# stoneMo/DeepAVFusion

Measured on AMD Instinct MI355X. Metric: AV-pairs/sec, DeepAVFusion ViT-B pre-training step (224px + 10s audio, image mask 0.75), higher is better.
Workload: dtype bf16; 1 GPU; AVMAE(DeepAVFusion base) fwd+bwd+allreduce+AdamW, B=64/GPU, 224x224 RGB + (128,640) log-mel, masks 0.75/0.8, fusion attn_ratio 0.25 mlp_ratio 1.0; global_batch=64, parallelism=dp1, graph=True

## Files before the change

### deepavfusion_amd/_lib.py

```python
from __future__ import annotations

import ctypes as C
import os

import torch

_HERE = os.path.dirname(os.path.abspath(__file__))
LIB_PATH = os.path.join(_HERE, 'libdavfusion_hip.so')

_p, _i, _l, _f, _sz = C.c_void_p, C.c_int, C.c_long, C.c_float, C.c_size_t

ABI_VERSION = 9

SIGNATURES = {
    'dav_abi_version': [],
    'dav_build_flags': [],
    'dav_last_error_string': [],
    'dav_tune': [_i, _i],
    'dav_gemm_nt_bf16': [_p, _p, _i, _i, _i, _i, _i, _p, _p, _i, _p, _i, _p, _i, _p, _p, _p, _i, _i, _p, _p, _i, _i, _i, _f, _i, _p],
    'dav_gemm_nt_ln_bf16': [_p, _p, _i, _i, _i, _i, _i, _p, _p, _i, _p, _i, _p, _i, _p, _p, _p, _i, _i, _p, _p, _i, _i, _i, _f, _i, _p, _p],
    'dav_ln_fold_grouped': [_p, _i, _p],
    'dav_rowstats_cast': [_p, _l, _i, _i, _i, _p, _p, _p],
    'dav_layernorm_bwd_twin': [_p, _l, _p, _i, _p, _l, _p, _i, _i, _i, _f, _p, _p, _p, _p,
                               _p, _l, _i, _p, _l, _p, _l,
                               _p, _l, _i, _p, _l, _p, _l,
                               _p, _p, _p, _p, _sz, _p],
    'dav_nt_issue_log': [_i, _p, _i],
    'dav_nt_tune_set': [_p, _i],
    'dav_gemm_tn_bf16': [_p, _p, _i, _i, _i, _i, _i, _p, _p, _p, _i, _i, _p, _i, _p],
    'dav_gemm_tn_grouped_bf16': [_p, _i, _p],
    'dav_gemm_tn_gang_workspace_bytes': [_p, _i],
    'dav_gemm_tn_gang_bf16': [_p, _i, _p, _sz, _p],
    'dav_gemm_tn_grouped_bf16_gated': [_p, _i, _p, _p],
    'dav_gemm_tn_gang_bf16_gated': [_p, _i, _p, _sz, _p, _p],
    'dav_attn_fwd': [_p, _p, _p, _p, _p, _i, _i, _i, _i, _i, _i, _l, _i, _l, _i, _l, _i, _l, _i, _f, _p],
    'dav_attn_bwd': [_p] * 10 + [_i] * 6 + [_l, _i] * 8 + [_f, _p],
    'dav_attn_bwd_part': [_p] * 10 + [_i] * 6 + [_l, _i] * 8 + [_f, _i, _p],
    'dav_add_cast': [_p, _p, _p, _p, _l, _p],
    'dav_attn_bwd_ctx': [_p] * 10 + [_i] * 6 + [_l, _i] * 8 + [_f, _i, _i, _p],
    'dav_attn_bias_fwd': [_p, _p, _p, _p, _p, _i, _i, _i, _i, _i, _i, _l, _i, _l, _i, _l, _i, _l, _i, _f, _p, _i, _i, _p],
    'dav_attn_bias_bwd': [_p] * 10 + [_i] * 6 + [_l, _i] * 8 + [_f, _p, _i, _i, _p, _i, _p],
    'dav_attn_drop_fwd': [_p, _p, _p, _p, _p, _i, _i, _i, _i, _i, _i, _l, _i, _l, _i, _l, _i, _l, _i, _f, _p, _i, _f, _p],
    'dav_attn_drop_bwd': [_p] * 10 + [_i] * 6 + [_l, _i] * 8 + [_f, _p, _i, _f, _i, _i, _p],
    'dav_window_unfold': [_p, _i, _p, _i, _i, _i, _i, _i, _i, _f, _p, _i, _p],
    'dav_window_fold': [_p, _p, _p, _i, _i, _i, _i, _i, _i, _f, _p, _p],
    'dav_relpos_bias_build': [_p, _p, _p, _i, _i, _i, _i, _i, _f, _p, _p],
    'dav_relpos_bias_bwd': [_p, _p, _i, _i, _i, _i, _i, _i, _p, _p],
    'dav_layernorm_fwd': [_p, _l, _i, _p, _l, _i, _i, _i, _p, _p, _f, _p, _p, _p, _p, _p],
    'dav_layernorm_bwd': [_p, _l, _i, _p, _l, _i, _i, _i, _p, _p, _p, _p, _p,
                          _p, _l, _i, _p, _l, _p, _l,
                          _p, _l, _i, _p, _l, _p, _l,
                          _p, _p, _p, _sz, _p],
    'dav_layernorm_bwd_workspace_bytes': [_i, _i],
    'dav_layernorm_bwd_reduce_grouped': [_p, _i, _p],
    'dav_mask_build': [_p, _i, _i, _i, _p, _p, _p, _p, _p, _p],
    'dav_patch_gather': [_p, _i, _i, _i, _i, _p, _i, _p, _p],
    'dav_patch_gather3d': [_p, _i, _i, _i, _i, _i, _i, _p, _i, _p, _p],
    'dav_unshuffle_fwd': [_p, _p, _p, _p, _i, _i, _i, _i, _p, _l, _i, _p],
    'dav_rows_gather_cast': [_p, _l, _i, _p, _i, _i, _i, _p, _p],
    'dav_rows_axpy': [_p, _p, _p, _i, _i, _i, _p, _p],
    'dav_rows_scale_cast': [_p, _p, _i, _i, _i, _p, _p],
    'dav_dropout_rows': [_p, _i, _p, _p, _f, _p, _i, _i, _i, _p, _i, _p],
    'dav_unshuffle_bwd_reduce': [_p, _l, _i, _p, _i, _i, _i, _i, _p, _p, _p],
    'dav_patch_mse_fwd': [_p, _p, _p, _i, _i, _i, _i, _i, _p, _p, _p, _p, _p, _p],
    'dav_patch_mse_bwd': [_p, _p, _p, _p, _p, _p, _p, _i, _i, _i, _i, _p, _p],
    'dav_pair_expand': [_p, _p, _i, _i, _i, _i, _p, _p],
    'dav_pair_reduce': [_p, _i, _i, _i, _i, _p, _p, _p],
# ... 27 lines not shown
    'dav_batch_suspend': [_i],
    'dav_batch_end': [],
    'dav_batch_abort': [],
    'dav_batch_stats': [_p, _p],
    'dav_adamw_flat': [_p, _p, _p, _p, _p, _l, _p, _p, _i, _f, _f, _f, _p, _f, _p, _i, _p, _p, _p],
    'dav_step_guard': [_p, _p, _p, _f, _f, _p, _p, _p],
    'dav_cast_transpose_grouped': [_p, _i, _p],
}

class DavLnReduce(C.Structure):
    _fields_ = [('workspace', C.c_void_p), ('dgamma', C.c_void_p), ('dbeta', C.c_void_p), ('rows', C.c_int), ('D', C.c_int)]


class DavNtLn(C.Structure):
    _fields_ = [('stats', C.c_void_p), ('stats2', C.c_void_p), ('A2', C.c_void_p), ('ln_c', C.c_void_p), ('eps', C.c_float),
                ('a_r0', C.c_int), ('a_r1', C.c_int), ('stats_out', C.c_void_p), ('twin_out', C.c_void_p), ('ld_twin', C.c_int)]


class DavLnFold(C.Structure):
    _fields_ = [('w', C.c_void_p), ('gamma', C.c_void_p), ('beta', C.c_void_p), ('bias', C.c_void_p),
                ('w_ln_bf16', C.c_void_p), ('ln_c', C.c_void_p), ('ln_d', C.c_void_p), ('N', C.c_int), ('K', C.c_int)]


class DavTranspose(C.Structure):
    _fields_ = [('x', C.c_void_p), ('y_bf16', C.c_void_p), ('R', C.c_int), ('C', C.c_int)]


class DavTnProblem(C.Structure):
    _fields_ = [('A', C.c_void_p), ('B', C.c_void_p), ('C', C.c_void_p), ('bias_grad', C.c_void_p),
                ('Mc', C.c_int), ('N', C.c_int), ('K', C.c_int), ('lda', C.c_int), ('ldb', C.c_int), ('ldc', C.c_int),
                ('a_rowmap', C.c_int * 3), ('b_rowmap', C.c_int * 3), ('flags', C.c_int)]


ERRORS = {-1: 'bad shape', -2: 'unsupported dtype', -3: 'insufficient workspace', -4: 'HIP error', -5: 'misaligned pointer/stride'}

_lib = None


def load():
    global _lib
    if _lib is not None:
        return _lib
    if not os.path.exists(LIB_PATH):
        raise RuntimeError(f'{LIB_PATH} is missing: the DeepAVFusion HIP kernels are not built '
                           '(run __graft_entry__.build() or make -C deepavfusion_amd/csrc). There is no CPU fallback.')
    lib = C.CDLL(LIB_PATH)
    for name, argtypes in SIGNATURES.items():
        fn = getattr(lib, name)
        fn.argtypes = argtypes
        fn.restype = _sz if name.endswith('workspace_bytes') else (C.c_char_p if name == 'dav_last_error_string' else _i)
    if lib.dav_abi_version() != ABI_VERSION:
        raise RuntimeError('libdavfusion_hip.so ABI version mismatch')
    _lib = lib
    load_nt_tuning(NT_TUNING_PATH)
    return lib


def kernel_source_hash():
    import glob
    import hashlib
    here = os.path.dirname(os.path.abspath(__file__))
    h = hashlib.sha1()
    for f in sorted(glob.glob(os.path.join(here, 'csrc', '*.hip')) + glob.glob(os.path.join(here, 'csrc', '*.h'))) + [os.path.join(here, 'tuning', 'nt_gfx950.json')]:
        h.update(os.path.basename(f).encode())
        h.update(open(f, 'rb').read())
    return h.hexdigest()[:16]
# ... 29 lines not shown
```

### deepavfusion_amd/csrc/accum/gemm_tn_gated.hip

```cpp
#include "../gemm.hip"

namespace {

static_assert(sizeof(TGWrite) + sizeof(const int*) <= 4096, "kernel argument block");
constexpr int TG_BETA_WORD = (int)(offsetof(TNParams, beta) / 4), TG_PROB_WORDS = (int)(sizeof(TNParams) / 4);

__global__ __launch_bounds__(64) void gemm_tn_gang_write_gated_kernel(const TGWrite w, const int* __restrict__ write_gate) {
  TGHeader* hd = reinterpret_cast<TGHeader*>(w.ws);
  TNParams* probs = reinterpret_cast<TNParams*>(w.ws + sizeof(TGHeader));
  TGDesc* desc = reinterpret_cast<TGDesc*>(w.ws + sizeof(TGHeader) + (size_t)w.count_total * sizeof(TNParams));
  const int b = blockIdx.x, t = threadIdx.x;
  if (b < w.item_count) {
    const TGItem it = w.item[b];
    const int nr = it.nrnc >> 16, nc = it.nrnc & 0xffff, r0 = it.r0c0 >> 16, c0 = it.r0c0 & 0xffff;
    for (int i = t; i < nr * nc; i += 64) desc[it.desc_first + i] = TGDesc{it.prob, ((r0 + i / nc) << 16) | (c0 + i % nc)};
    return;
  }
  const bool closed = write_gate[0] == 0;
  const int* src = reinterpret_cast<const int*>(w.prob);
  int* dst = reinterpret_cast<int*>(probs + w.prob_first);
  for (int i = t; i < w.prob_count * TG_PROB_WORDS; i += 64) dst[i] = (closed && i % TG_PROB_WORDS == TG_BETA_WORD) ? 1 : src[i];
  if (w.write_header) {
    if (t < 8) hd->head[t] = 0;
    if (t < 9) hd->q_start[t] = w.q_start[t];
// ... 86 lines not shown
  for (int i = 0; i < count; ++i) {
    if (w.prob_count == TG_WCH) { flush(); reset(i); }
    const DavTnProblem& q = probs[i];
    TNParams& p = w.prob[w.prob_count++];
    p.A = (const bf16_t*)q.A; p.B = (const bf16_t*)q.B; p.Mc = q.Mc; p.N = q.N; p.K = q.K; p.lda = q.lda; p.ldb = q.ldb;
    p.amap = RowMap{q.a_rowmap[0], q.a_rowmap[1], q.a_rowmap[2]};
    p.bmap = RowMap{q.b_rowmap[0], q.b_rowmap[1], q.b_rowmap[2]};
    p.C = q.C; p.ldc = q.ldc; p.beta = (q.flags & 1) ? 0 : 1; p.bias_grad = q.bias_grad; p.debug_plain_store = 0; p.splits = 1;
    for (const TGPlanItem* it : by_prob[i]) {
      if (w.item_count == TG_WIT) { flush(); reset(i + 1); }
      w.item[w.item_count++] = TGItem{i, q_start[it->queue] + it->first, (it->r0 << 16) | it->c0, (it->nr << 16) | it->nc};
    }
  }
  flush();
  static std::mutex dev_mu;
  static int dev_cus[64] = {0};
  int n_wg = 256;
  {
    int dev = 0;
    if (hipGetDevice(&dev) != hipSuccess || dev < 0 || dev >= 64) return DAV_ERR_HIP;
    std::lock_guard<std::mutex> lk(dev_mu);
    if (!dev_cus[dev]) {
      if (hipFuncSetAttribute((const void*)gemm_tn_gang_kernel, hipFuncAttributeMaxDynamicSharedMemorySize, 160 * 1024) != hipSuccess) return DAV_ERR_HIP;
      int cus = 256;
      (void)hipDeviceGetAttribute(&cus, hipDeviceAttributeMultiprocessorCount, dev);
      dev_cus[dev] = cus > 0 ? cus : 256;
    }
    n_wg = dev_cus[dev];
  }
  const int grid = (int)std::min<long>(n_wg, (long)q_start[8]);
  DAV_LAUNCH(gemm_tn_gang_kernel, dim3(grid), dim3(512), TNG_LDS, stream, (char*)workspace, count, dbg);
  return dav_launch_status();
}
```

### deepavfusion_amd/engine.py

```python
from __future__ import annotations

import os
from typing import Callable, Dict, List, Optional

import torch

from . import ops
from .ops import F32

BF16 = torch.bfloat16
PRECISION = 'bf16'


def set_precision(p: str):
    global BF16, PRECISION
    if p not in ('bf16', 'fp32'):
        raise ValueError(p)
    PRECISION = p
    BF16 = torch.float32 if p == 'fp32' else torch.bfloat16

_GRAD_READY: Optional[Callable[[torch.nn.Parameter], None]] = None


def set_grad_ready_hook(fn: Optional[Callable[[torch.nn.Parameter], None]]):
# ... 324 lines not shown
            _FOLD_PENDING.clear()
            _FOLD_JOINED.clear()
        _FOLD_SCOPE = self.prev
        return False


class region:

    def __enter__(self):
        self.own = None
        if _BATCH is not None:
            ops.batch_region(True)
        elif batching_allowed():
            self.own = batch(auto_lanes=True)
            self.own.__enter__()
        return self

    def __exit__(self, et, ev, tb):
        if self.own is not None:
            return self.own.__exit__(et, ev, tb)
        if _BATCH is not None and et is None:
            ops.batch_region(False)
        return False


WGRAD_GANG = os.environ.get('DAV_WGRAD_GANG', '1') != '0'
WGRAD_GANG_MIN_TILES = 512
WGRAD_MERGE = int(os.environ.get('DAV_WGRAD_MERGE', '0'))
WGRAD_FLUSH_LAYERS = None


WGRAD_EAGER_DP_MERGE = 3


def wgrad_flush_due(layer: int, depth: int) -> bool:
    if not WGRAD_GANG or layer == 0 or layer in (WGRAD_FLUSH_LAYERS or ()):
        return True
    if WGRAD_MERGE > 0:
        return (depth - layer) % WGRAD_MERGE == 0
    return _GRAD_READY is not None and WGRAD_FLUSH_LAYERS is None and (depth - layer) % WGRAD_EAGER_DP_MERGE == 0


_DEFERRED = None
_DEFERRED_LN = None
_DEFERRED_LN_READY = []


class deferred_wgrads:
    def __enter__(self):
        global _DEFERRED, _DEFERRED_LN
        self.prev = (_DEFERRED, _DEFERRED_LN)
        _DEFERRED, _DEFERRED_LN = [], []
        return self

    def __exit__(self, *exc):
        global _DEFERRED, _DEFERRED_LN
        if exc[0] is None:
            flush_wgrads()
        _DEFERRED, _DEFERRED_LN = self.prev


_OVERWRITE = None


def wgrad_overwrite_begin(gate=None):
    global _OVERWRITE
    _OVERWRITE = dict(written=set(), touched=set(), params={}, gate=gate)


def wgrad_overwrite_end():
    global _OVERWRITE
    st, _OVERWRITE = _OVERWRITE, None
    return list(st['params'].values()) if st else []


def deferred_operands_to(stream):
    for pr in (_DEFERRED or []):
        for k in ('A', 'B'):
            t = pr.get(k)
            if torch.is_tensor(t) and t.is_cuda:
                t.record_stream(stream)
    for item in (_DEFERRED_LN or []):
        if torch.is_tensor(item[0]) and item[0].is_cuda:
            item[0].record_stream(stream)


def flush_wgrads():
    if _DEFERRED_LN:
        items = list(_DEFERRED_LN)
        del _DEFERRED_LN[:]
        ops.layernorm_bwd_reduce_grouped(items)
        for pair in _DEFERRED_LN_READY:
            _ready(*pair)
        del _DEFERRED_LN_READY[:]
    if not _DEFERRED:
        return
    probs = list(_DEFERRED)
    del _DEFERRED[:]
    while probs:
        seen, now, later = set(), [], []
        for pr in probs:
            key = pr['C'].data_ptr()
            (later if key in seen else now).append(pr)
            seen.add(key)
        now.sort(key=lambda pr: -pr['Mc'])
        gate = _OVERWRITE['gate'] if _OVERWRITE is not None else None
        gated = {} if gate is None else {'gate': gate}
        gang = WGRAD_GANG and PRECISION == 'bf16' and (sum(-(-pr['N'] // 256) * -(-pr['K'] // 256) for pr in now) >= WGRAD_GANG_MIN_TILES
                                                       or any(pr['Mc'] % 64 for pr in now))
        if _OVERWRITE is not None:
            for pr in now:
                key = pr['C'].data_ptr()
                pr['overwrite'] = bool(pr.get('weight') is not None and key not in _OVERWRITE['written'] and key not in _OVERWRITE['touched'])
                if gate is not None and (pr['A'].dtype == F32 or (not gang and pr['Mc'] % 64)):
                    pr['overwrite'] = False
                _OVERWRITE['written'].add(key)
                if pr.get('weight') is None:
                    _OVERWRITE['touched'].add(pr.get('gbase', key))
                if pr['overwrite']:
                    _OVERWRITE['params'][id(pr['weight'])] = pr['weight']
        if gang:
            ops.gemm_tn_gang(now, **gated)
        else:
            grouped = [pr for pr in now if pr['Mc'] % 64 == 0 or pr['A'].dtype == F32]
            if grouped:
                ops.gemm_tn_grouped(grouped, **gated)
            for pr in now:
                if pr['Mc'] % 64 and pr['A'].dtype != F32:
                    ops.gemm_tn(pr['A'], pr['B'], pr['Mc'], pr['N'], pr['K'], pr['C'], lda=pr['lda'], ldb=pr['ldb'], ldc=pr['ldc'],
                                a_rowmap=pr.get('a_rowmap'), b_rowmap=pr.get('b_rowmap'), beta=0 if pr.get('overwrite') else 1,
                                bias_grad=pr.get('bias_grad'))
        for pr in now:
            _ready(*pr['ready'])
        probs = later


def ln_fwd(norm, x0, x1, B, eps=None, want_f32=False, want_bf16=True):
    D = norm.weight.shape[0]
    r0 = x0.shape[1] if x0 is not None else 0
    r1 = x1.shape[1] if x1 is not None else 0
    if x0 is None:
        x0, r0, x1, r1 = x1, r1, None, 0
    dev = x0.device
    M = B * (r0 + r1)
    y = _e((M, D), BF16, dev) if want_bf16 else None
    y32 = _e((M, D), F32, dev) if want_f32 else None
    if PRECISION == 'fp32' and y is not None and y32 is not None:
        y32 = y
    mean, rstd = _e((M,), F32, dev), _e((M,), F32, dev)
    ops.layernorm_fwd(x0, r0 * D, r0, x1, r1 * D, r1, B, D, norm.weight, norm.bias, norm.eps if eps is None else eps,
                      y, y32, mean, rstd)
    return y, y32, (mean, rstd)


# ... 854 lines not shown
    else:
        got = (img.shape[2] // pt) * (img.shape[3] // 16) * (img.shape[4] // 16)
        if tuple(img.shape[2:]) != tuple(pe.input_size):
            raise RuntimeError(f'The size of tensor a ({got}) must match the size of tensor b ({L}) at non-singleton dimension 1')
    if C != pe.proj.weight.shape[1]:
        raise RuntimeError(f'Given groups=1, weight of size {list(pe.proj.weight.shape)}, expected input{list(img.shape)} to have '
                           f'{pe.proj.weight.shape[1]} channels, but got {C} channels instead')
    if clip and nk != L:
        raise RuntimeError(f'The size of tensor a ({nk}) must match the size of tensor b ({L}) at non-singleton dimension 1')
    K = C * pt * 256
    A = _e((B * nk, K), BF16, img.device)
    ops.patch_gather(img, ids_keep32, nk, A, pt)
    Wb = wcache(pe.proj.weight)
    tok = _e((B, nk, D), F32, img.device)
    pos_by_id = ids_keep32 is not None and not clip
    if ln_fuse_ok(D) and K % 64 == 0:
        tw = (_e((B * nk, D), BF16, img.device), _e((B * nk, D // 64, 2), F32, img.device))
        ops.gemm_nt_ln(A, Wb, B * nk, D, K, prod=dict(stats_out=tw[1], twin_out=tw[0], ld_twin=D), bias=pe.proj.bias, res=vit.pos_embed,
                       ldres=D, res_rows=ids_keep32 if pos_by_id else None, res_rowmap=None if pos_by_id else (L, 0, 0), C_out=tok)
        tw_set(tok, *tw)
    else:
        ops.gemm_nt(A, Wb, B * nk, D, K, bias=pe.proj.bias, res=vit.pos_embed, ldres=D,
                    res_rows=ids_keep32 if pos_by_id else None, res_rowmap=None if pos_by_id else (L, 0, 0), C_out=tok)
    return tok, dict(A=A, nk=nk)


def patch_embed_bwd(vit, t, g, gb):
    pe = vit.patch_embed
    D = vit.embed_dim
    A = t['A']
    M, K = A.shape
    if gb is None:
        gb = to_bf16(g)
    ops.gemm_tn(gb, A, M, D, K, gbuf(pe.proj.weight).view(D, K), beta=1, bias_grad=gbuf(pe.proj.bias))
    _ready(pe.proj.weight, pe.proj.bias)


def drain(steps):
    try:
        while True:
            next(steps)
    except StopIteration as e:
        return e.value


def decoder_fwd(dec, x_b, xf_b, ids_restore32, B, nk, nF):
    return drain(decoder_fwd_steps(dec, x_b, xf_b, ids_restore32, B, nk, nF))


def decoder_fwd_steps(dec, x_b, xf_b, ids_restore32, B, nk, nF):
    L = ids_restore32.shape[1]
    Dd = dec.embed.weight.shape[0]
    dev = x_b.device
    emb = lin_fwd(dec.embed, x_b, B * nk)
    x = _e((B, nF + L, Dd), F32, dev)
    lin_fwd(dec.embed, xf_b, B * nF, out=x, c_rowmap=(nF, nF + L, 0))
    ops.unshuffle_fwd(emb, dec.mask_token, dec.pos_embed, ids_restore32, B, L, nk, Dd, x, (nF + L) * Dd, nF)
    tapes = []
    swin = getattr(dec, 'arch', 'plain') == 'swin'
    for blk in dec.blocks:
        if swin:
            x, bt = swin_block_fwd(blk, x, nF)
        else:
            x, bt = block_fwd(blk, x, None, dec.heads, blk.norm1.eps)
        tapes.append(bt)
        yield
# ... 152 lines not shown
```

### deepavfusion_amd/ops.py

```python
from __future__ import annotations

import ctypes as C
from typing import Optional, Sequence

import torch

from . import _lib

BF16 = torch.bfloat16
F32 = torch.float32


def _stream():
    return torch.cuda.current_stream().cuda_stream


import threading

_TLS = threading.local()


def hold(*tensors):
    h = getattr(_TLS, 'hold', None)
    if h is not None:
# ... 197 lines not shown
            continue
        _lib.check(lib.dav_gemm_tn_grouped_bf16(_tn_problem_array(chunk), len(chunk), _stream()), 'dav_gemm_tn_grouped_bf16')


def _tn_problem_array(problems):
    arr = (_lib.DavTnProblem * len(problems))()
    for q, d in zip(arr, problems):
        q.A, q.B, q.C, q.bias_grad = _ptr(d['A']), _ptr(d['B']), _ptr(d['C']), _ptr(d.get('bias_grad'))
        q.Mc, q.N, q.K, q.lda, q.ldb, q.ldc = d['Mc'], d['N'], d['K'], d['lda'], d['ldb'], d['ldc']
        q.a_rowmap[:] = d.get('a_rowmap') or (0, 0, 0)
        q.b_rowmap[:] = d.get('b_rowmap') or (0, 0, 0)
        q.flags = 1 if d.get('overwrite') else 0
    return arr


def gemm_tn_gang(problems, workspace_fill=None, gate=None):
    if not problems:
        return
    if problems[0]['A'].dtype == F32:
        return gemm_tn_grouped(problems) if gate is None else gemm_tn_grouped(problems, gate)
    lib = _lib.load()
    arr = _tn_problem_array(problems)
    nbytes = int(lib.dav_gemm_tn_gang_workspace_bytes(arr, len(problems)))
    if nbytes == 0:
        raise RuntimeError('dav_gemm_tn_gang_workspace_bytes: invalid weight-gradient problem (shape / alignment)')
    ws = torch.empty(nbytes, dtype=torch.uint8, device=problems[0]['A'].device)
    if workspace_fill is not None:
        ws.fill_(workspace_fill)
    hold(ws)
    if gate is not None:
        _lib.check(lib.dav_gemm_tn_gang_bf16_gated(arr, len(problems), _ptr(ws), nbytes, _gate_ptr(gate), _stream()), 'dav_gemm_tn_gang_bf16_gated')
        return
    _lib.check(lib.dav_gemm_tn_gang_bf16(arr, len(problems), _ptr(ws), nbytes, _stream()), 'dav_gemm_tn_gang_bf16')


def attn_fwd(q_ptr, k_ptr, v_ptr, O, LSE, B, H, Nq, Nk, dqk, dv, q_bs, q_rs, k_bs, k_rs, v_bs, v_rs, o_bs, o_rs, scale):
    lib = _lib.load()
    if O.dtype == F32:
        _lib.check(lib.dav_attn_fwd_f32(q_ptr, k_ptr, v_ptr, _ptr(O), _ptr(LSE), B, H, Nq, Nk, dqk, dv, q_bs, q_rs, k_bs, k_rs,
                                        v_bs, v_rs, o_bs, o_rs, float(scale), _stream()), 'dav_attn_fwd_f32')
        return
    _lib.check(lib.dav_attn_fwd(q_ptr, k_ptr, v_ptr, _ptr(O), _ptr(LSE), B, H, Nq, Nk, dqk, dv, q_bs, q_rs, k_bs, k_rs,
                                v_bs, v_rs, o_bs, o_rs, float(scale), _stream()), 'dav_attn_fwd')


def attn_bias_fwd(q_ptr, k_ptr, v_ptr, O, LSE, B, H, Nq, Nk, dqk, dv, q_bs, q_rs, k_bs, k_rs, v_bs, v_rs, o_bs, o_rs, scale,
                  bias, bias_nb, bias_ld):
    lib = _lib.load()
    fn, name = (lib.dav_attn_bias_fwd_f32, 'dav_attn_bias_fwd_f32') if O.dtype == F32 else (lib.dav_attn_bias_fwd, 'dav_attn_bias_fwd')
    _lib.check(fn(q_ptr, k_ptr, v_ptr, _ptr(O), _ptr(LSE), B, H, Nq, Nk, dqk, dv, q_bs, q_rs, k_bs, k_rs, v_bs, v_rs, o_bs, o_rs,
                  float(scale), _ptr(bias), bias_nb, bias_ld, _stream()), name)


def attn_bias_bwd(q_ptr, k_ptr, v_ptr, O, dO, LSE, Delta, dq_ptr, dk_ptr, dv_ptr, B, H, Nq, Nk, dqk, dv, q_bs, q_rs, k_bs, k_rs,
                  v_bs, v_rs, o_bs, o_rs, do_bs, do_rs, dq_bs, dq_rs, dk_bs, dk_rs, dv_bs, dv_rs, scale, bias, bias_nb, bias_ld,
                  dS, part=3):
    lib = _lib.load()
    fn, name = (lib.dav_attn_bias_bwd_f32, 'dav_attn_bias_bwd_f32') if O.dtype == F32 else (lib.dav_attn_bias_bwd, 'dav_attn_bias_bwd')
    _lib.check(fn(q_ptr, k_ptr, v_ptr, _ptr(O), _ptr(dO), _ptr(LSE), _ptr(Delta), dq_ptr, dk_ptr, dv_ptr, B, H, Nq, Nk, dqk, dv,
                  q_bs, q_rs, k_bs, k_rs, v_bs, v_rs, o_bs, o_rs, do_bs, do_rs, dq_bs, dq_rs, dk_bs, dk_rs, dv_bs, dv_rs,
                  float(scale), _ptr(bias), bias_nb, bias_ld, _ptr(dS), part, _stream()), name)


def window_unfold(src, rows32, B, nW, A, nF, L, Cc, fusion_scale, out):
    _lib.check(_lib.load().dav_window_unfold(_ptr(src), int(src.dtype == BF16), _ptr(rows32), B, nW, A, nF, L, Cc, float(fusion_scale),
                                             _ptr(out), int(out.dtype == BF16), _stream()), 'dav_window_unfold')
# ... 354 lines not shown
```

### deepavfusion_amd/util/misc.py

```python
from __future__ import annotations

import contextlib
import copy
import math
import os

import torch

from .. import engine, ops
from . import distributed as dist_utils
from .flat import FlatAdamW


def get_grad_norm_(parameters, norm_type: float = 2.0) -> torch.Tensor:
    if isinstance(parameters, torch.Tensor):
        parameters = [parameters]
    grads = [p.grad.detach() for p in parameters if p.grad is not None]
    if not grads:
        return torch.tensor(0.)
    if norm_type == math.inf:
        return max(g.abs().max() for g in grads)
    return torch.norm(torch.stack([torch.norm(g, norm_type) for g in grads]), norm_type)


# ... 183 lines not shown
        cap = torch.cuda.Stream()
        cap.wait_stream(torch.cuda.current_stream())
        self.opt.flat.zero_grad()
        self.keep_grad = torch.zeros_like(self.opt.keep_grad)
        self.step_scale = torch.ones(1, dtype=torch.float32, device=dev)
        self.bad_steps = torch.zeros(1, dtype=torch.int32, device=dev)
        self._presq = torch.zeros(1, dtype=torch.float32, device=dev)
        self._presq_ws = torch.zeros(1024, dtype=torch.float32, device=dev)
        accum = self.accum_iter > 1
        self.gate = torch.ones(1, dtype=torch.int32, device=dev) if accum else None
        self._sums_dirty = False
        if accum:
            self.loss_sum_image = torch.zeros((), dtype=torch.float32, device=dev)
            self.loss_sum_audio = torch.zeros((), dtype=torch.float32, device=dev)
            self.grad_norm = torch.zeros(1, dtype=torch.float32, device=dev)
        gscale = 1.0 / self.accum_iter

        def optimizer_pass():
            gnorm = None
            if self.clip_grad is not None:
                ops.l2norm(self.opt.flat.flat_g, self._presq, self._presq_ws, 1.0)
                gnorm = self._presq
            if not accum:
                ops.step_guard(self.loss_image, self.loss_audio, gnorm, self.clip_grad, 1.0, self.step_scale, self.bad_steps)
                self.opt.launch_step(fused_norm_and_zero=True, keep_grad=self.keep_grad, gscale_dev=self.step_scale)
                self.grad_norm = self.opt.sumsq.sqrt()
                return
            ops.step_guard(self.loss_sum_image, self.loss_sum_audio, gnorm, self.clip_grad, gscale, self.step_scale, self.bad_steps)
            self.opt.launch_step(grad_scale=gscale, fused_norm_and_zero=True, keep_grad=self.keep_grad, gscale_dev=self.step_scale)
            torch.mul(self.opt.sumsq.sqrt(), gscale, out=self.grad_norm)
            self.loss_sum_image.zero_()
            self.loss_sum_audio.zero_()
        kept = set()
        with torch.cuda.stream(cap):
            self.graphs[0].capture_begin(capture_error_mode=CAPTURE_MODE)
            try:
                if os.environ.get('DAV_WGRAD_OVERWRITE', '1') != '0':
                    engine.wgrad_overwrite_begin(self.gate)
                engine.WGRAD_FLUSH_LAYERS = set(self.cuts)
                engine.invalidate_weight_cache(self.model.parameters())
                engine.refresh_weight_cache(self.model)
                self.loss_image, self.loss_audio = self._fwd_bwd(layer_cb)
                if accum:
                    self.loss_sum_image.add_(self.loss_image.reshape(()))
                    self.loss_sum_audio.add_(self.loss_audio.reshape(()))
            finally:
                kept = {id(p) for p in engine.wgrad_overwrite_end()}
                engine.WGRAD_FLUSH_LAYERS = None
            if not self.dist_active and not accum:
                optimizer_pass()
            self.graphs[seg[0]].capture_end()
            self.opt_graph = None
            if self.dist_active or accum:
                self.opt_graph = torch.cuda.CUDAGraph()
                self.opt_graph.capture_begin(pool=self.graphs[0].pool(), capture_error_mode=CAPTURE_MODE)
                optimizer_pass()
                self.opt_graph.capture_end()
        torch.cuda.current_stream().wait_stream(cap)
        torch.cuda.synchronize()
        if self.reducer is not None:
            done = {bi for s in self.bucket_sched for bi in s}
            self.bucket_sched[-1] += [bi for bi in range(len(self.reducer.buckets)) if bi not in done]
        engine.set_grad_ready_hook(saved_hook)
        self.opt.flat.zero_grad()
        self.keep_grad.copy_(torch.tensor([1 if id(p) in kept else 0 for p in self.opt.flat.params], dtype=torch.uint8))
        self.kept_params = len(kept)

    def check(self):
        n = int(self.bad_steps.item())
        if n:
            raise RuntimeError(f'Loss is {float(self.loss_image + self.loss_audio)}, stopping training '
                               f'({n} captured step(s) had a non-finite loss or gradient norm; their updates were skipped)')

    def _fwd_bwd(self, layer_cb):
        B, dev = self.image.shape[0], self.image.device
        Li, La = self.model.image_gs[0] * self.model.image_gs[1], self.model.audio_gs[0] * self.model.audio_gs[1]
        if self.inject_noise:
            noise_i, noise_a = self.noise_image, self.noise_audio
        else:
            noise_i, noise_a = torch.rand(B, Li, device=dev), torch.rand(B, La, device=dev)
        with engine.ln_fuse_for(True):
            outs, tape, aux = self.bridge.avmae_fwd(self.model, self.image, self.audio, noise_i, noise_a)
        one = torch.ones((), device=dev)
        self.bridge.avmae_bwd(self.model, tape, one, one, layer_cb=layer_cb)
        return outs[0], outs[1]

    def __call__(self, image, audio, noise_image=None, noise_audio=None):
        self.image.copy_(image, non_blocking=True)
        self.audio.copy_(audio, non_blocking=True)
        if self.inject_noise:
            self.noise_image.copy_(noise_image, non_blocking=True)
            self.noise_audio.copy_(noise_audio, non_blocking=True)
        elif noise_image is not None or noise_audio is not None:
            raise ValueError('masking noise given to a step captured with inject_noise=False (it draws its own inside the graph)')
        if self.accum_iter == 1:
            self.opt.prepare_step()
            if self.reducer is not None:
                self.reducer.begin_backward()
            for s, g in enumerate(self.graphs):
                g.replay()
                if self.reducer is not None and self.dist_active:
                    self.reducer.launch_buckets(self.bucket_sched[s])
            if self.opt_graph is not None:
                self.reducer.finish()
                self.opt_graph.replay()
            self.opt.flat.stale = self.kept_params > 0
            engine.bump_fold_generation()
            self.tr.n_steps += 1
            return self.loss_image, self.loss_audio, self.grad_norm
        tr = self.tr
        write_first, reduce, optimize = micro_step_plan(tr.accums, self.accum_iter, self.dist_active)
        if write_first and self._sums_dirty:
            self.loss_sum_image.zero_()
            self.loss_sum_audio.zero_()
        self.gate.fill_(1 if write_first else 0)
        reduce = reduce and self.dist_active
        if self.reducer is not None:
# ... 85 lines not shown
```

### include/dav_kernels.h

```cpp
#ifndef DAV_KERNELS_H_
#define DAV_KERNELS_H_

#include <stddef.h>
#include <stdint.h>

#ifdef __HIPCC__
#include <hip/hip_runtime.h>
#else
typedef struct ihipStream_t* hipStream_t;
#endif

#ifdef __cplusplus
extern "C" {
#endif

#define DAV_ABI_VERSION 9
int dav_abi_version(void);
int dav_build_flags(void);
const char* dav_last_error_string(void);
int dav_tune(int knob, int value);

int dav_gemm_nt_bf16(const void* A, const void* B, int M, int N, int K, int lda, int ldb, const int* a_rowmap,
                     const float* bias, int act, const void* aux, int ldaux, const float* res, int ldres,
                     const int* res_rowmap, const int* res_rows, void* C, int ldc, int c_is_bf16, const int* c_rowmap,
                     void* C2, int ldc2, int c2_mode, int beta, float alpha, int variant, hipStream_t stream);

typedef struct DavNtLn {
  const float* stats; const float* stats2; const void* A2; const float* ln_c; float eps; int a_r0, a_r1;
  float* stats_out; void* twin_out; int ld_twin;
} DavNtLn;
int dav_gemm_nt_ln_bf16(const void* A, const void* B, int M, int N, int K, int lda, int ldb, const int* a_rowmap,
                        const float* bias, int act, const void* aux, int ldaux, const float* res, int ldres,
                        const int* res_rowmap, const int* res_rows, void* C, int ldc, int c_is_bf16, const int* c_rowmap,
                        void* C2, int ldc2, int c2_mode, int beta, float alpha, int variant, const DavNtLn* ln, hipStream_t stream);

int dav_nt_issue_log(int enable, int* out, int capacity);

int dav_nt_tune_set(const int* blob, int n_ints);

int dav_gemm_tn_bf16(const void* A, const void* B, int Mc, int N, int K, int lda, int ldb, const int* a_rowmap,
                     const int* b_rowmap, float* C, int ldc, int beta, float* bias_grad, int variant, hipStream_t stream);

typedef struct DavTnProblem {
  const void* A; const void* B;
  float* C; float* bias_grad;
  int Mc, N, K, lda, ldb, ldc;
  int a_rowmap[3], b_rowmap[3];
  int flags;
} DavTnProblem;
int dav_gemm_tn_grouped_bf16(const DavTnProblem* problems, int count, hipStream_t stream);

size_t dav_gemm_tn_gang_workspace_bytes(const DavTnProblem* problems, int count);
int dav_gemm_tn_gang_bf16(const DavTnProblem* problems, int count, void* workspace, size_t workspace_bytes, hipStream_t stream);

int dav_gemm_tn_grouped_bf16_gated(const DavTnProblem* problems, int count, const int* write_gate, hipStream_t stream);
int dav_gemm_tn_gang_bf16_gated(const DavTnProblem* problems, int count, void* workspace, size_t workspace_bytes, const int* write_gate,
                                hipStream_t stream);

int dav_attn_fwd(const void* Q, const void* K, const void* V, void* O, float* LSE, int B, int H, int Nq, int Nk, int dqk,
                 int dv, long q_bs, int q_rs, long k_bs, int k_rs, long v_bs, int v_rs, long o_bs, int o_rs, float scale,
                 hipStream_t stream);
int dav_attn_bwd(const void* Q, const void* K, const void* V, const void* O, const void* dO, const float* LSE, float* Delta,
                 void* dQ, void* dK, void* dV, int B, int H, int Nq, int Nk, int dqk, int dv, long q_bs, int q_rs, long k_bs,
                 int k_rs, long v_bs, int v_rs, long o_bs, int o_rs, long do_bs, int do_rs, long dq_bs, int dq_rs, long dk_bs,
                 int dk_rs, long dv_bs, int dv_rs, float scale, hipStream_t stream);
int dav_attn_bwd_part(const void* Q, const void* K, const void* V, const void* O, const void* dO, const float* LSE, float* Delta,
                 void* dQ, void* dK, void* dV, int B, int H, int Nq, int Nk, int dqk, int dv, long q_bs, int q_rs, long k_bs,
                 int k_rs, long v_bs, int v_rs, long o_bs, int o_rs, long do_bs, int do_rs, long dq_bs, int dq_rs, long dk_bs,
                 int dk_rs, long dv_bs, int dv_rs, float scale, int part, hipStream_t stream);

int dav_attn_bwd_ctx(const void* Q, const void* K, const void* V, const void* O, const void* dO, const float* LSE, float* Delta,
                 void* dQ, void* dK, void* dV, int B, int H, int Nq, int Nk, int dqk, int dv, long q_bs, int q_rs, long k_bs,
                 int k_rs, long v_bs, int v_rs, long o_bs, int o_rs, long do_bs, int do_rs, long dq_bs, int dq_rs, long dk_bs,
                 int dk_rs, long dv_bs, int dv_rs, float scale, int dq_ctx_rows, int part, hipStream_t stream);

int dav_attn_bias_fwd(const void* Q, const void* K, const void* V, void* O, float* LSE, int B, int H, int Nq, int Nk, int dqk,
                      int dv, long q_bs, int q_rs, long k_bs, int k_rs, long v_bs, int v_rs, long o_bs, int o_rs, float scale,
                      const float* bias, int bias_nb, int bias_ld, hipStream_t stream);
int dav_attn_bias_bwd(const void* Q, const void* K, const void* V, const void* O, const void* dO, const float* LSE, float* Delta,
                      void* dQ, void* dK, void* dV, int B, int H, int Nq, int Nk, int dqk, int dv, long q_bs, int q_rs, long k_bs,
                      int k_rs, long v_bs, int v_rs, long o_bs, int o_rs, long do_bs, int do_rs, long dq_bs, int dq_rs, long dk_bs,
                      int dk_rs, long dv_bs, int dv_rs, float scale, const float* bias, int bias_nb, int bias_ld, float* dS,
                      int part, hipStream_t stream);

int dav_attn_drop_fwd(const void* Q, const void* K, const void* V, void* O, float* LSE, int B, int H, int Nq, int Nk, int dqk,
                      int dv, long q_bs, int q_rs, long k_bs, int k_rs, long v_bs, int v_rs, long o_bs, int o_rs, float scale,
                      const void* keep, int keep_ld, float keep_scale, hipStream_t stream);
int dav_attn_drop_bwd(const void* Q, const void* K, const void* V, const void* O, const void* dO, const float* LSE, float* Delta,
                      void* dQ, void* dK, void* dV, int B, int H, int Nq, int Nk, int dqk, int dv, long q_bs, int q_rs, long k_bs,
                      int k_rs, long v_bs, int v_rs, long o_bs, int o_rs, long do_bs, int do_rs, long dq_bs, int dq_rs, long dk_bs,
// ... 141 lines not shown
```

Measured before the change: 2607 AV-pairs/s.

## Defer all weight-gradient GEMMs into one prepared gang launch per captured step

During graph capture in the single-device, non-accumulating case, all deferred weight-gradient GEMMs (including patch-embed) are held back until the end of backward. Problems sharing the same weight are joined into a two-segment problem chained through the splits field. The gang's descriptor tables are written once outside the graph, so the captured graph holds only a persistent run kernel that resets its queue counters on exit. The aim is to cut per-layer table-write and launch overhead and fill the GPU with one large batch of tiles. In exchange, weight-gradient work no longer overlaps earlier in backward, and correctness now depends on the workspace staying intact across replays.

```diff
diff --git a/deepavfusion_amd/_lib.py b/deepavfusion_amd/_lib.py
--- a/deepavfusion_amd/_lib.py
+++ b/deepavfusion_amd/_lib.py
@@ -33,6 +33,10 @@
     'dav_gemm_tn_gang_bf16': [_p, _i, _p, _sz, _p],
     'dav_gemm_tn_grouped_bf16_gated': [_p, _i, _p, _p],
     'dav_gemm_tn_gang_bf16_gated': [_p, _i, _p, _sz, _p, _p],
+    'dav_gemm_tn_gang_size': [_p, _p, _i, _p],
+    'dav_gemm_tn_gang_prepare': [_p, _p, _i, _p, _sz, _p],
+    'dav_gemm_tn_gang_run': [_p, _p, _i, _p, _sz, _p],
+    'dav_gemm_tn_gang2_bf16': [_p, _p, _i, _p, _sz, _p],
     'dav_attn_fwd': [_p, _p, _p, _p, _p, _i, _i, _i, _i, _i, _i, _l, _i, _l, _i, _l, _i, _l, _i, _f, _p],
     'dav_attn_bwd': [_p] * 10 + [_i] * 6 + [_l, _i] * 8 + [_f, _p],
     'dav_attn_bwd_part': [_p] * 10 + [_i] * 6 + [_l, _i] * 8 + [_f, _i, _p],
@@ -126,6 +130,11 @@
                 ('a_rowmap', C.c_int * 3), ('b_rowmap', C.c_int * 3), ('flags', C.c_int)]
 
 
+class DavTnSegment(C.Structure):
+    _fields_ = [('A', C.c_void_p), ('B', C.c_void_p), ('Mc', C.c_int), ('lda', C.c_int), ('ldb', C.c_int),
+                ('a_rowmap', C.c_int * 3), ('b_rowmap', C.c_int * 3)]
+
+
 ERRORS = {-1: 'bad shape', -2: 'unsupported dtype', -3: 'insufficient workspace', -4: 'HIP error', -5: 'misaligned pointer/stride'}
 
 _lib = None
diff --git a/deepavfusion_amd/csrc/accum/gemm_tn_gated.hip b/deepavfusion_amd/csrc/accum/gemm_tn_gated.hip
--- a/deepavfusion_amd/csrc/accum/gemm_tn_gated.hip
+++ b/deepavfusion_amd/csrc/accum/gemm_tn_gated.hip
@@ -142,3 +142,5 @@
   DAV_LAUNCH(gemm_tn_gang_kernel, dim3(grid), dim3(512), TNG_LDS, stream, (char*)workspace, count, dbg);
   return dav_launch_status();
 }
+
+#include "../wgrad/gemm_tn_prepared.h"
diff --git a/deepavfusion_amd/csrc/wgrad/gemm_tn_prepared.h b/deepavfusion_amd/csrc/wgrad/gemm_tn_prepared.h
--- /dev/null
+++ b/deepavfusion_amd/csrc/wgrad/gemm_tn_prepared.h
@@ -0,0 +1,194 @@
+#pragma once
+
+namespace {
+
+__global__ __launch_bounds__(64) void gemm_tn_gang_exit_clear_kernel(char* ws) {
+  if (threadIdx.x == 0) reinterpret_cast<TGHeader*>(ws)->pad[0] = 0;
+}
+
+__global__ __launch_bounds__(512) void gemm_tn_gang_run_kernel(char* __restrict__ ws, const int entries, const int dbg) {
+  extern __shared__ __attribute__((aligned(16))) char smem[];
+  TGHeader* hd = reinterpret_cast<TGHeader*>(ws);
+  const int* probs = reinterpret_cast<const int*>(ws + sizeof(TGHeader));
+  const TGDesc* desc = reinterpret_cast<const TGDesc*>(ws + sizeof(TGHeader) + (size_t)entries * sizeof(TNParams));
+  volatile __attribute__((address_space(3))) int* slot = (volatile __attribute__((address_space(3))) int*)(smem + NT256_LDS);
+  int xcd;
+  asm volatile("s_getreg_b32 %0, hwreg(HW_REG_XCC_ID)" : "=s"(xcd));
+  xcd &= 7;
+  if (dbg & 8) xcd = blockIdx.x & 7;
+  if (dbg & 16) xcd = (blockIdx.x >> 5) & 7;
+  for (int a = 0; a < 8; ++a) {
+    const int q = (xcd + a) & 7;
+    const int qs = hd->q_start[q], qn = hd->q_start[q + 1] - qs;
+    while (true) {
+      if (threadIdx.x == 0) {
+        const int t = __hip_atomic_load(&hd->head[q], __ATOMIC_RELAXED, __HIP_MEMORY_SCOPE_AGENT) >= qn
+                          ? qn : __hip_atomic_fetch_add(&hd->head[q], 1, __ATOMIC_RELAXED, __HIP_MEMORY_SCOPE_AGENT);
+        *slot = t;
+      }
+      __syncthreads();
+      const int t = __builtin_amdgcn_readfirstlane(*slot);
+      __syncthreads();
+      if (t >= qn) break;
+      const TGDesc d = desc[qs + t];
+      const int bnbk = __builtin_amdgcn_readfirstlane(d.bnbk);
+      int pi = __builtin_amdgcn_readfirstlane(d.prob);
+      while (true) {
+        union { TNParams p; int w[sizeof(TNParams) / 4]; } u;
+#pragma unroll
+        for (int i = 0; i < (int)(sizeof(TNParams) / 4); ++i) u.w[i] = __builtin_amdgcn_readfirstlane(probs[pi * (int)(sizeof(TNParams) / 4) + i]);
+        tng_tile(u.p, bnbk >> 16, bnbk & 0xffff, dbg);
+        pi = u.p.splits;
+        if (pi <= 0 || pi >= entries) break;
+      }
+    }
+  }
+  if (threadIdx.x == 0) {
+    const int left = __hip_atomic_fetch_add(&hd->pad[0], 1, __ATOMIC_ACQ_REL, __HIP_MEMORY_SCOPE_AGENT);
+    if (left == (int)gridDim.x - 1) {
+      for (int q = 0; q < 8; ++q) __hip_atomic_store(&hd->head[q], 0, __ATOMIC_RELAXED, __HIP_MEMORY_SCOPE_AGENT);
+      __hip_atomic_store(&hd->pad[0], 0, __ATOMIC_RELEASE, __HIP_MEMORY_SCOPE_AGENT);
+    }
+  }
+}
+
+struct TGTables {
+  std::vector<TNParams> entries;
+  std::vector<TGPlanItem> items;
+  int q_start[9];
+  int count;
+  size_t bytes() const { return sizeof(TGHeader) + entries.size() * sizeof(TNParams) + (size_t)q_start[8] * sizeof(TGDesc); }
+};
+
+int tn_gang2_tables(const DavTnProblem* probs, const DavTnSegment* second, int count, TGTables& t) {
+  if (!probs) return DAV_ERR_SHAPE;
+  const int chk = tn_gang_check(probs, count);
+  if (chk != DAV_OK) return chk;
+  std::vector<DavTnProblem> whole(probs, probs + count);
+  for (int i = 0; second && i < count; ++i) {
+    const DavTnSegment& s = second[i];
+    if (s.Mc < 0) return DAV_ERR_SHAPE;
+    if (s.Mc == 0) continue;
+    if (!s.A || !s.B || (s.lda & 7) || (s.ldb & 7) || (long)s.Mc + probs[i].Mc > 0x7fffffffL) return DAV_ERR_SHAPE;
+    if (((uintptr_t)s.A | (uintptr_t)s.B) & 15) return DAV_ERR_ALIGN;
+    whole[i].Mc += s.Mc;
+  }
+  tn_gang_plan(whole.data(), count, t.items, t.q_start);
+  t.count = count;
+  t.entries.clear();
+  for (int i = 0; i < count; ++i) {
+    const DavTnProblem& q = probs[i];
+    TNParams p;
+    p.A = (const bf16_t*)q.A; p.B = (const bf16_t*)q.B; p.Mc = q.Mc; p.N = q.N; p.K = q.K; p.lda = q.lda; p.ldb = q.ldb;
+    p.amap = RowMap{q.a_rowmap[0], q.a_rowmap[1], q.a_rowmap[2]};
+    p.bmap = RowMap{q.b_rowmap[0], q.b_rowmap[1], q.b_rowmap[2]};
+    p.C = q.C; p.ldc = q.ldc; p.beta = (q.flags & 1) ? 0 : 1; p.bias_grad = q.bias_grad; p.debug_plain_store = 0; p.splits = 0;
+    t.entries.push_back(p);
+  }
+  for (int i = 0; second && i < count; ++i) {
+    const DavTnSegment& s = second[i];
+    if (s.Mc == 0) continue;
+    TNParams p = t.entries[i];
+    p.A = (const bf16_t*)s.A; p.B = (const bf16_t*)s.B; p.Mc = s.Mc; p.lda = s.lda; p.ldb = s.ldb;
+    p.amap = RowMap{s.a_rowmap[0], s.a_rowmap[1], s.a_rowmap[2]};
+    p.bmap = RowMap{s.b_rowmap[0], s.b_rowmap[1], s.b_rowmap[2]};
+    p.beta = 1;
+    t.entries[i].splits = (int)t.entries.size();
+    t.entries.push_back(p);
+  }
+  return DAV_OK;
+}
+
+int tn_gang2_write(const TGTables& t, void* workspace, hipStream_t stream) {
+  const int total = (int)t.entries.size();
+  bool header = true;
+  std::vector<std::vector<const TGPlanItem*>> by_prob(t.count);
+  for (const TGPlanItem& it : t.items) by_prob[it.prob].push_back(&it);
+  TGWrite w;
+  auto reset = [&](int first) {
+    w.ws = (char*)workspace; w.prob_first = first; w.prob_count = 0; w.item_count = 0; w.count_total = total; w.write_header = 0;
+    for (int q = 0; q < 9; ++q) w.q_start[q] = t.q_start[q];
+  };
+  auto flush = [&]() {
+    if (!w.prob_count && !w.item_count && !header) return;
+    w.write_header = header ? 1 : 0; header = false;
+    const TGWrite wl = w;
+    DAV_LAUNCH(gemm_tn_gang_write_kernel, dim3(wl.item_count + 1), dim3(64), 0, stream, wl);
+  };
+  reset(0);
+  for (int i = 0; i < total; ++i) {
+    if (w.prob_count == TG_WCH) { flush(); reset(i); }
+    w.prob[w.prob_count++] = t.entries[i];
+    if (i >= t.count) continue;
+    for (const TGPlanItem* it : by_prob[i]) {
+      if (w.item_count == TG_WIT) { flush(); reset(i + 1); }
+      w.item[w.item_count++] = TGItem{i, t.q_start[it->queue] + it->first, (it->r0 << 16) | it->c0, (it->nr << 16) | it->nc};
+    }
+  }
+  flush();
+  DAV_LAUNCH(gemm_tn_gang_exit_clear_kernel, dim3(1), dim3(64), 0, stream, (char*)workspace);
+  return dav_launch_status();
+}
+
+int tn_gang2_launch(const TGTables& t, void* workspace, hipStream_t stream) {
+  static const int dbg = getenv("DAV_TN_GANG_DEBUG") ? atoi(getenv("DAV_TN_GANG_DEBUG")) & 24 : 0;
+  static std::mutex dev_mu;
+  static int dev_cus[64] = {0};
+  int n_wg = 256;
+  {
+    int dev = 0;
+    if (hipGetDevice(&dev) != hipSuccess || dev < 0 || dev >= 64) return DAV_ERR_HIP;
+    std::lock_guard<std::mutex> lk(dev_mu);
+    if (!dev_cus[dev]) {
+      if (hipFuncSetAttribute((const void*)gemm_tn_gang_run_kernel, hipFuncAttributeMaxDynamicSharedMemorySize, 160 * 1024) != hipSuccess) return DAV_ERR_HIP;
+      int cus = 256;
+      (void)hipDeviceGetAttribute(&cus, hipDeviceAttributeMultiprocessorCount, dev);
+      dev_cus[dev] = cus > 0 ? cus : 256;
+    }
+    n_wg = dev_cus[dev];
+  }
+  const int grid = (int)std::min<long>(n_wg, (long)t.q_start[8]);
+  DAV_LAUNCH(gemm_tn_gang_run_kernel, dim3(grid), dim3(512), TNG_LDS, stream, (char*)workspace, (int)t.entries.size(), dbg);
+  return dav_launch_status();
+}
+
+int tn_gang2_entry(const DavTnProblem* probs, const DavTnSegment* second, int count, void* workspace, size_t workspace_bytes, hipStream_t stream,
+                   bool write, bool launch) {
+  if (!probs || !workspace) return DAV_ERR_SHAPE;
+  TGTables t;
+  const int chk = tn_gang2_tables(probs, second, count, t);
+  if (chk != DAV_OK) return chk;
+  if ((uintptr_t)workspace & 15) return DAV_ERR_ALIGN;
+  if (workspace_bytes < t.bytes()) return DAV_ERR_WORKSPACE;
+  if (write) {
+    const int rc = tn_gang2_write(t, workspace, stream);
+    if (rc != DAV_OK) return rc;
+  }
+  return launch ? tn_gang2_launch(t, workspace, stream) : DAV_OK;
+}
+
+}
+
+extern "C" int dav_gemm_tn_gang_size(const DavTnProblem* probs, const DavTnSegment* second, int count, size_t* workspace_bytes) {
+  if (!probs || !workspace_bytes) return DAV_ERR_SHAPE;
+  TGTables t;
+  const int chk = tn_gang2_tables(probs, second, count, t);
+  if (chk != DAV_OK) return chk;
+  *workspace_bytes = t.bytes();
+  return DAV_OK;
+}
+
+extern "C" int dav_gemm_tn_gang_prepare(const DavTnProblem* probs, const DavTnSegment* second, int count, void* workspace, size_t workspace_bytes,
+                                        hipStream_t stream) {
+  return tn_gang2_entry(probs, second, count, workspace, workspace_bytes, stream, true, false);
+}
+
+extern "C" int dav_gemm_tn_gang_run(const DavTnProblem* probs, const DavTnSegment* second, int count, void* workspace, size_t workspace_bytes,
+                                    hipStream_t stream) {
+  return tn_gang2_entry(probs, second, count, workspace, workspace_bytes, stream, false, true);
+}
+
+extern "C" int dav_gemm_tn_gang2_bf16(const DavTnProblem* probs, const DavTnSegment* second, int count, void* workspace, size_t workspace_bytes,
+                                      hipStream_t stream) {
+  return tn_gang2_entry(probs, second, count, workspace, workspace_bytes, stream, true, true);
+}
diff --git a/deepavfusion_amd/engine.py b/deepavfusion_amd/engine.py
--- a/deepavfusion_amd/engine.py
+++ b/deepavfusion_amd/engine.py
@@ -380,8 +380,64 @@
 
 WGRAD_EAGER_DP_MERGE = 3
 
+WGRAD_ONE_LAUNCH = True
+WGRAD_JOIN = True
+WGRAD_PREPARED = True
+WGRAD_CAPTURE = None
+
+
+def wgrad_capture_begin(workspace=None):
+    global WGRAD_CAPTURE
+    WGRAD_CAPTURE = dict(one_launch=bool(WGRAD_ONE_LAUNCH and WGRAD_GANG), join=bool(WGRAD_JOIN and WGRAD_GANG),
+                         prepared=[] if (WGRAD_PREPARED and WGRAD_GANG and workspace is not None) else None)
+    if WGRAD_CAPTURE['prepared'] is not None:
+        WGRAD_CAPTURE.update(workspace=workspace, used=0)
+    return WGRAD_CAPTURE
+
+
+def wgrad_workspace_bytes(params) -> int:
+    total = 4096
+    for p in params:
+        if p.ndim >= 2:
+            N = p.shape[0]
+            total += 16 * 96 + 8 * 2 * -(-N // 256) * (-(-(p.numel() // N) // 256) + 16)
+    return total
+
+
+def wgrad_capture_end():
+    global WGRAD_CAPTURE
+    WGRAD_CAPTURE = None
+
+
+def wgrad_hold_back() -> bool:
+    return WGRAD_CAPTURE is not None and WGRAD_CAPTURE['one_launch'] and PRECISION == 'bf16'
+
+
+def _join_same_weight(probs):
+    by_c = {}
+    for pr in probs:
+        by_c.setdefault(pr['C'].data_ptr(), []).append(pr)
+    out, dropped = [], set()
+    for pr in probs:
+        if id(pr) in dropped:
+            continue
+        grp = by_c[pr['C'].data_ptr()]
+        if len(grp) == 2 and grp[0] is pr:
+            a, b = grp
+            bga, bgb = a.get('bias_grad'), b.get('bias_grad')
+            same_bias = (bga is None and bgb is None) or (bga is not None and bgb is not None and bga.data_ptr() == bgb.data_ptr())
+            if (a['A'].dtype == BF16 and b['A'].dtype == BF16 and same_bias and a.get('weight') is b.get('weight')
+                    and all(a[k] == b[k] for k in ('N', 'K', 'ldc'))):
+                pr = dict(a, second=dict(A=b['A'], B=b['B'], Mc=b['Mc'], lda=b['lda'], ldb=b['ldb'], a_rowmap=b.get('a_rowmap'),
+                                         b_rowmap=b.get('b_rowmap')), ready=tuple(a['ready']) + tuple(b['ready']))
+                dropped.add(id(b))
+        out.append(pr)
+    return out
+
 
 def wgrad_flush_due(layer: int, depth: int) -> bool:
+    if wgrad_hold_back() and _DEFERRED is not None:
+        return False
     if not WGRAD_GANG or layer == 0 or layer in (WGRAD_FLUSH_LAYERS or ()):
         return True
     if WGRAD_MERGE > 0:
@@ -398,12 +454,14 @@
     def __enter__(self):
         global _DEFERRED, _DEFERRED_LN
         self.prev = (_DEFERRED, _DEFERRED_LN)
-        _DEFERRED, _DEFERRED_LN = [], []
+        self.shared = _DEFERRED is not None and wgrad_hold_back()
+        if not self.shared:
+            _DEFERRED, _DEFERRED_LN = [], []
         return self
 
     def __exit__(self, *exc):
         global _DEFERRED, _DEFERRED_LN
-        if exc[0] is None:
+        if exc[0] is None and not self.shared:
             flush_wgrads()
         _DEFERRED, _DEFERRED_LN = self.prev
 
@@ -431,6 +489,12 @@
     for item in (_DEFERRED_LN or []):
         if torch.is_tensor(item[0]) and item[0].is_cuda:
             item[0].record_stream(stream)
+
+
+def _gang_worthy(now) -> bool:
+    return bool(WGRAD_GANG and PRECISION == 'bf16'
+                and (sum(-(-pr['N'] // 256) * -(-pr['K'] // 256) for pr in now) >= WGRAD_GANG_MIN_TILES
+                     or any(pr['Mc'] % 64 or (pr.get('second') or {}).get('Mc', 0) % 64 for pr in now)))
 
 
 def flush_wgrads():
@@ -443,8 +507,15 @@
         del _DEFERRED_LN_READY[:]
     if not _DEFERRED:
         return
+    if wgrad_hold_back():
+        deferred_operands_to(torch.cuda.current_stream())
     probs = list(_DEFERRED)
     del _DEFERRED[:]
+    cap = WGRAD_CAPTURE if (_OVERWRITE is None or _OVERWRITE['gate'] is None) and PRECISION == 'bf16' else None
+    if cap is not None and cap['join']:
+        joined = _join_same_weight(probs)
+        if _gang_worthy(joined):
+            probs = joined
     while probs:
         seen, now, later = set(), [], []
         for pr in probs:
@@ -454,8 +525,8 @@
         now.sort(key=lambda pr: -pr['Mc'])
         gate = _OVERWRITE['gate'] if _OVERWRITE is not None else None
         gated = {} if gate is None else {'gate': gate}
-        gang = WGRAD_GANG and PRECISION == 'bf16' and (sum(-(-pr['N'] // 256) * -(-pr['K'] // 256) for pr in now) >= WGRAD_GANG_MIN_TILES
-                                                       or any(pr['Mc'] % 64 for pr in now))
+        gang = _gang_worthy(now)
+        assert gang or not any(pr.get('second') for pr in now)
         if _OVERWRITE is not None:
             for pr in now:
                 key = pr['C'].data_ptr()
@@ -467,7 +538,15 @@
                     _OVERWRITE['touched'].add(pr.get('gbase', key))
                 if pr['overwrite']:
                     _OVERWRITE['params'][id(pr['weight'])] = pr['weight']
-        if gang:
+        if gang and cap is not None and cap['prepared'] is not None:
+            ws = cap['workspace'][cap['used']:]
+            pg = ops.PreparedGang(now, ws=ws)
+            cap['used'] += -(-pg.nbytes // 256) * 256
+            pg.run()
+            cap['prepared'].append(pg)
+        elif gang and any(pr.get('second') for pr in now):
+            ops.gemm_tn_gang2(now)
+        elif gang:
             ops.gemm_tn_gang(now, **gated)
         else:
             grouped = [pr for pr in now if pr['Mc'] % 64 == 0 or pr['A'].dtype == F32]
@@ -1388,6 +1467,11 @@
     M, K = A.shape
     if gb is None:
         gb = to_bf16(g)
+    if wgrad_hold_back() and _DEFERRED is not None and D % 8 == 0 and K % 8 == 0 and gb.dtype == BF16:
+        gw = gbuf(pe.proj.weight).view(D, K)
+        _DEFERRED.append(dict(A=gb, B=A, Mc=M, N=D, K=K, C=gw, lda=D, ldb=K, ldc=K, a_rowmap=None, b_rowmap=None,
+                              bias_grad=gbuf(pe.proj.bias), ready=(pe.proj.weight, pe.proj.bias), gbase=gw.data_ptr(), weight=pe.proj.weight))
+        return
     ops.gemm_tn(gb, A, M, D, K, gbuf(pe.proj.weight).view(D, K), beta=1, bias_grad=gbuf(pe.proj.bias))
     _ready(pe.proj.weight, pe.proj.bias)
 
diff --git a/deepavfusion_amd/ops.py b/deepavfusion_amd/ops.py
--- a/deepavfusion_amd/ops.py
+++ b/deepavfusion_amd/ops.py
@@ -253,6 +253,57 @@
         _lib.check(lib.dav_gemm_tn_gang_bf16_gated(arr, len(problems), _ptr(ws), nbytes, _gate_ptr(gate), _stream()), 'dav_gemm_tn_gang_bf16_gated')
         return
     _lib.check(lib.dav_gemm_tn_gang_bf16(arr, len(problems), _ptr(ws), nbytes, _stream()), 'dav_gemm_tn_gang_bf16')
+
+
+def _tn_segment_array(problems):
+    if not any(d.get('second') for d in problems):
+        return None
+    arr = (_lib.DavTnSegment * len(problems))()
+    for q, d in zip(arr, problems):
+        s = d.get('second')
+        if not s:
+            continue
+        q.A, q.B, q.Mc, q.lda, q.ldb = _ptr(s['A']), _ptr(s['B']), s['Mc'], s['lda'], s['ldb']
+        q.a_rowmap[:] = s.get('a_rowmap') or (0, 0, 0)
+        q.b_rowmap[:] = s.get('b_rowmap') or (0, 0, 0)
+    return arr
+
+
+class PreparedGang:
+
+    def __init__(self, problems, workspace_fill=None, ws=None):
+        if not problems or problems[0]['A'].dtype == F32:
+            raise RuntimeError('PreparedGang: bf16 weight-gradient problems only')
+        self.lib = _lib.load()
+        self.problems = list(problems)
+        self.arr, self.seg, self.count = _tn_problem_array(problems), _tn_segment_array(problems), len(problems)
+        nbytes = C.c_size_t(0)
+        _lib.check(self.lib.dav_gemm_tn_gang_size(self.arr, self.seg, self.count, C.byref(nbytes)), 'dav_gemm_tn_gang_size')
+        self.nbytes = int(nbytes.value)
+        if ws is not None:
+            if ws.dtype != torch.uint8 or ws.numel() < self.nbytes:
+                raise RuntimeError(f'PreparedGang: the workspace given holds {ws.numel()} bytes, the tables need {self.nbytes}')
+            self.ws = ws
+        elif torch.cuda.is_current_stream_capturing():
+            raise RuntimeError('PreparedGang: a launch recorded in a graph needs a workspace allocated outside the capture')
+        else:
+            self.ws = torch.empty(self.nbytes, dtype=torch.uint8, device=problems[0]['A'].device)
+        if workspace_fill is not None:
+            self.ws.fill_(workspace_fill)
+
+    def prepare(self):
+        _lib.check(self.lib.dav_gemm_tn_gang_prepare(self.arr, self.seg, self.count, _ptr(self.ws), self.nbytes, _stream()), 'dav_gemm_tn_gang_prepare')
+
+    def run(self):
+        _lib.check(self.lib.dav_gemm_tn_gang_run(self.arr, self.seg, self.count, _ptr(self.ws), self.nbytes, _stream()), 'dav_gemm_tn_gang_run')
+
+
+def gemm_tn_gang2(problems, workspace_fill=None):
+    if not problems:
+        return
+    pg = PreparedGang(problems, workspace_fill)
+    hold(pg.ws)
+    _lib.check(pg.lib.dav_gemm_tn_gang2_bf16(pg.arr, pg.seg, pg.count, _ptr(pg.ws), pg.nbytes, _stream()), 'dav_gemm_tn_gang2_bf16')
 
 
 def attn_fwd(q_ptr, k_ptr, v_ptr, O, LSE, B, H, Nq, Nk, dqk, dv, q_bs, q_rs, k_bs, k_rs, v_bs, v_rs, o_bs, o_rs, scale):
diff --git a/deepavfusion_amd/util/misc.py b/deepavfusion_amd/util/misc.py
--- a/deepavfusion_amd/util/misc.py
+++ b/deepavfusion_amd/util/misc.py
@@ -239,12 +239,16 @@
             self.loss_sum_image.zero_()
             self.loss_sum_audio.zero_()
         kept = set()
+        self.wgrad_plan = None
+        self._wgrad_ws = torch.empty(engine.wgrad_workspace_bytes(self.model.parameters()), dtype=torch.uint8, device=dev)
         with torch.cuda.stream(cap):
             self.graphs[0].capture_begin(capture_error_mode=CAPTURE_MODE)
             try:
                 if os.environ.get('DAV_WGRAD_OVERWRITE', '1') != '0':
                     engine.wgrad_overwrite_begin(self.gate)
                 engine.WGRAD_FLUSH_LAYERS = set(self.cuts)
+                if self.reducer is None and self.n_seg == 1 and not accum:
+                    self.wgrad_plan = engine.wgrad_capture_begin(self._wgrad_ws)
                 engine.invalidate_weight_cache(self.model.parameters())
                 engine.refresh_weight_cache(self.model)
                 self.loss_image, self.loss_audio = self._fwd_bwd(layer_cb)
@@ -254,6 +258,7 @@
             finally:
                 kept = {id(p) for p in engine.wgrad_overwrite_end()}
                 engine.WGRAD_FLUSH_LAYERS = None
+                engine.wgrad_capture_end()
             if not self.dist_active and not accum:
                 optimizer_pass()
             self.graphs[seg[0]].capture_end()
@@ -264,6 +269,9 @@
                 optimizer_pass()
                 self.opt_graph.capture_end()
         torch.cuda.current_stream().wait_stream(cap)
+        self.prepared_wgrads = list((self.wgrad_plan or {}).get('prepared') or [])
+        for pg in self.prepared_wgrads:
+            pg.prepare()
         torch.cuda.synchronize()
         if self.reducer is not None:
             done = {bi for s in self.bucket_sched for bi in s}
@@ -289,7 +297,8 @@
         with engine.ln_fuse_for(True):
             outs, tape, aux = self.bridge.avmae_fwd(self.model, self.image, self.audio, noise_i, noise_a)
         one = torch.ones((), device=dev)
-        self.bridge.avmae_bwd(self.model, tape, one, one, layer_cb=layer_cb)
+        with engine.deferred_wgrads() if engine.wgrad_hold_back() else contextlib.nullcontext():
+            self.bridge.avmae_bwd(self.model, tape, one, one, layer_cb=layer_cb)
         return outs[0], outs[1]
 
     def __call__(self, image, audio, noise_image=None, noise_audio=None):
diff --git a/include/dav_kernels.h b/include/dav_kernels.h
--- a/include/dav_kernels.h
+++ b/include/dav_kernels.h
@@ -56,6 +56,19 @@
 int dav_gemm_tn_grouped_bf16_gated(const DavTnProblem* problems, int count, const int* write_gate, hipStream_t stream);
 int dav_gemm_tn_gang_bf16_gated(const DavTnProblem* problems, int count, void* workspace, size_t workspace_bytes, const int* write_gate,
                                 hipStream_t stream);
+
+typedef struct DavTnSegment {
+  const void* A; const void* B;
+  int Mc, lda, ldb;
+  int a_rowmap[3], b_rowmap[3];
+} DavTnSegment;
+int dav_gemm_tn_gang_size(const DavTnProblem* problems, const DavTnSegment* second, int count, size_t* workspace_bytes);
+int dav_gemm_tn_gang_prepare(const DavTnProblem* problems, const DavTnSegment* second, int count, void* workspace, size_t workspace_bytes,
+                             hipStream_t stream);
+int dav_gemm_tn_gang_run(const DavTnProblem* problems, const DavTnSegment* second, int count, void* workspace, size_t workspace_bytes,
+                         hipStream_t stream);
+int dav_gemm_tn_gang2_bf16(const DavTnProblem* problems, const DavTnSegment* second, int count, void* workspace, size_t workspace_bytes,
+                           hipStream_t stream);
 
 int dav_attn_fwd(const void* Q, const void* K, const void* V, void* O, float* LSE, int B, int H, int Nq, int Nk, int dqk,
                  int dv, long q_bs, int q_rs, long k_bs, int k_rs, long v_bs, int v_rs, long o_bs, int o_rs, float scale,
```

Result: no change. 2630 AV-pairs/s, median of 6 (+0.9%).
